# AzureLeon1/DiffSpectra

Hardware: AMD Instinct MI355X
Metric: molecules/sec, 1000-step QM9S all-spectra sampling (partial run) (higher is better)
Workload: dtype f32 (GEMMs as split-fp16 x3 MFMA with fp32 accumulate; fp32-level accuracy, parity gates unchanged)

## Files before the change

### __graft_entry__.py

```python
from __future__ import annotations

import os
import subprocess
import sys

ROOT = os.path.dirname(os.path.abspath(__file__))
if ROOT not in sys.path:
    sys.path.insert(0, ROOT)

CSRC = os.path.join(ROOT, "diffspectra_amd", "csrc")
HIP_SOURCES = [os.path.join(CSRC, n) for n in ("ds_forward.hip", "ds_gemm.hip", "ds_sampler.hip", "ds_spec.hip", "ds_aux.hip", "ds_match.hip", "ds_graph.hip", "ds_mces.hip", "ds_morgan.hip", "ds_subgeom.hip", "ds_mmd.hip", "ds_sets.hip", "ds_valence.hip", "ds_train.hip", "ds_train_gemm.hip", "ds_train_attn.hip", "ds_train_chain.hip")]
HIP_DEPS = [os.path.join(CSRC, "ds_device.h"), os.path.join(CSRC, "ds_host.h"), os.path.join(CSRC, "ds_train_common.h"), os.path.join(CSRC, "ds_svd3.h"), os.path.join(CSRC, "ds_records.h"), os.path.join(CSRC, "ds_bonds.h"),
            os.path.join(ROOT, "include", "diffspectra_hip.h"), os.path.join(ROOT, "include", "diffspectra_train.h"),
            os.path.join(ROOT, "include", "diffspectra_sets.h"), os.path.join(ROOT, "include", "diffspectra_valence.h")]
LIB = os.path.join(ROOT, "diffspectra_amd", "libdiffspectra_hip.so")
OBJ_DIR = os.path.join(ROOT, "build", "obj")
BASE_FLAGS = ["--offload-arch=gfx950", "-O3", "-std=c++17", "-fPIC", "-Wno-pass-failed", "-Wno-unused-value"]
OPT_FLAGS = ["-mllvm", "-amdgpu-mfma-vgpr-form=1"]
LIBRARY_STATE = "not built"


def _digest(paths):
    import hashlib
    h = hashlib.sha1()
    for p in paths:
        h.update(os.path.basename(p).encode() + b"\0")
        with open(p, "rb") as f:
            h.update(f.read())
    return h.hexdigest()


def _read(path):
    try:
        with open(path) as f:
            return f.read()
    except OSError:
        return None


def _stale(target, deps):
    return not os.path.exists(target) or any(not os.path.exists(d) for d in deps) or _read(target + ".src") != _digest(deps)


def _compile(hipcc, src, obj, flags):
    cmd = [hipcc, *flags, "-c", src, "-o", obj]
    print("[build]", " ".join(cmd), file=sys.stderr, flush=True)
    r = subprocess.run(cmd, cwd=ROOT, capture_output=True, text=True)
    if r.returncode != 0 and "Unknown command line argument" in r.stderr and any(f in flags for f in OPT_FLAGS):
        flags = [f for f in flags if f not in OPT_FLAGS]
        print("[build] this hipcc does not know -amdgpu-mfma-vgpr-form; retrying without it", file=sys.stderr, flush=True)
        return _compile(hipcc, src, obj, flags)
    if r.returncode != 0:
        sys.stderr.write(r.stderr)
        raise subprocess.CalledProcessError(r.returncode, cmd)
    with open(obj + ".flags", "w") as f:
        f.write(" ".join(flags))
    with open(obj + ".src", "w") as f:
        f.write(_digest([src] + HIP_DEPS))


def build(force: bool = False) -> None:
    from concurrent.futures import ThreadPoolExecutor
    hipcc = os.environ.get("HIPCC", "/opt/rocm/bin/hipcc")
    flags = BASE_FLAGS + OPT_FLAGS
    sources = [s for s in HIP_SOURCES if os.path.exists(s)]
    os.makedirs(OBJ_DIR, exist_ok=True)
    objs = [os.path.join(OBJ_DIR, os.path.basename(s)[:-4] + ".o") for s in sources]
# ... 63 lines not shown
```

### diffspectra_amd/abi.py

```python
from __future__ import annotations

import ctypes as C
import os
import re
import struct as _struct
from typing import Dict, List, NamedTuple, Tuple

_INCLUDE = os.path.join(os.path.dirname(os.path.dirname(os.path.abspath(__file__))), "include")

_FIELD_CODES = {"int64_t": "q", "int32_t": "i", "uint32_t": "I", "uint64_t": "Q", "float": "f"}
_CTYPES = {"P": C.c_void_p, "q": C.c_int64, "i": C.c_int32, "I": C.c_uint32, "Q": C.c_uint64, "f": C.c_float}
_ARG_CTYPES = {"*": C.c_void_p, "int": C.c_int, "int32_t": C.c_int32, "int64_t": C.c_int64, "uint32_t": C.c_uint32, "uint64_t": C.c_uint64,
               "float": C.c_float, "double": C.c_double}


class Prototype(NamedTuple):
    name: str
    ret: str
    params: List[Tuple[str, str]]

    @property
    def argtypes(self):
        return [_ARG_CTYPES[t] for _, t in self.params]

# ... 32 lines not shown
        self.prototypes = {name: Prototype(name, ret, self._params(name, params))
                           for ret, name, params in re.findall(r"^\s*(int|void)\s+(\w+)\s*\(([^()]*)\)\s*;", self.text, flags=re.M)}

    def _fields(self, body: str) -> List[Tuple[str, str]]:
        fields = []
        for decl in filter(None, (d.strip() for d in body.split(";"))):
            typ, rest = re.fullmatch(r"(?:const\s+)?(\w+)\s*(.*)", decl, flags=re.S).groups()
            for f_ in rest.split(","):
                name, length = re.fullmatch(r"([*\s]*\w+)\s*(?:\[\s*(\w+)\s*\])?", f_.strip()).groups()
                code = "P" if name.startswith("*") else _FIELD_CODES[typ]
                if length is not None:
                    code = f"{self.consts[length] if length in self.consts else int(length)}{code}"
                fields.append((name.lstrip("* "), code))
        return fields

    @staticmethod
    def _params(function: str, text: str) -> List[Tuple[str, str]]:
        params = []
        if text.strip() == "void":
            return params
        for decl in (d.strip() for d in text.split(",")):
            if "*" in decl:
                typ, m = "*", re.fullmatch(r"[\w\s*]*?(\w+)", decl)
            else:
                m = re.fullmatch(r"(?:const\s+)?(\w+)\s+(\w+)", decl)
                typ, m = (m.group(1), m) if m else (None, None)
            if m is None or typ not in _ARG_CTYPES:
                raise ValueError(f"{function}: parameter '{decl}' is neither a pointer nor one of the scalar types {sorted(_ARG_CTYPES)[1:]}")
            params.append((m.group(m.lastindex), typ))
        return params

    def exports(self, prefix: str) -> List[str]:
        return [name for name in self.prototypes if name.startswith(prefix)]

    def bind(self, lib: C.CDLL) -> None:
        for p in self.prototypes.values():
            fn = getattr(lib, p.name)
            fn.restype = None if p.ret == "void" else C.c_int
            fn.argtypes = p.argtypes

    def packer(self, name: str) -> _struct.Struct:
        return _struct.Struct("@" + "".join(code for _, code in self.structs[name]))

    def ctypes_struct(self, name: str):
        def ctype(code):
            return _CTYPES[code[-1]] * int(code[:-1]) if len(code) > 1 else _CTYPES[code]
        return type(name, (C.Structure,), {"_fields_": [(f_, ctype(code)) for f_, code in self.structs[name]]})


SAMPLING = Header("diffspectra_hip.h")
TRAINING = Header("diffspectra_train.h")
SETS = Header("diffspectra_sets.h")
VALENCE = Header("diffspectra_valence.h")
```

### diffspectra_amd/csrc/ds_forward.hip

```cpp
#include <hip/hip_runtime.h>
#include <math.h>
#include <stdint.h>
#include <stdlib.h>

#include <atomic>
#include <mutex>
#include <utility>
#include <vector>

#include "../../include/diffspectra_hip.h"
#include "ds_device.h"
#include "ds_host.h"

#define ADAC DS_ADA_COLS
constexpr int DS_NODE_PF = 8;
constexpr int DS_NODE_PF2 = 4;
constexpr int DS_QKV_PF = 4;
constexpr int DS_TWO_STREAM_MAX_PAIRS = 400000;

#ifdef DS_STAMPS
#define DS_STAMP_INIT()                                                                                 \
  unsigned long long _sa[16] = {0, 0, 0, 0, 0, 0, 0, 0, 0, 0, 0, 0, 0, 0, 0, 0};                        \
  unsigned long long _t0 = __builtin_amdgcn_s_memtime()
#define DS_STAMP(i)                                                                                     \
  do {                                                                                                  \
    const unsigned long long _t1 = __builtin_amdgcn_s_memtime();                                        \
    _sa[i] += _t1 - _t0;                                                                                \
    _t0 = _t1;                                                                                          \
  } while (0)
#define DS_STAMP_W(i)                                                                                   \
  do {                                                                                                  \
    asm volatile("s_waitcnt vmcnt(0) lgkmcnt(0)" ::: "memory");                                         \
    DS_STAMP(i);                                                                                        \
  } while (0)
#define DS_STAMP_FLUSH(t)                                                                               \
  do {                                                                                                  \
    if (threadIdx.x == (t))                                                                             \
      for (int _i = 0; _i < 16; ++_i)                                                                   \
        if (_sa[_i]) atomicAdd(reinterpret_cast<unsigned long long*>(c.ws.flags + 16) + _i, _sa[_i]);   \
  } while (0)
#else
#define DS_STAMP_INIT()
#define DS_STAMP(i)
#define DS_STAMP_W(i)
#define DS_STAMP_FLUSH(t)
#endif

namespace {

using dst::clear;
using dst::record;
using dst::wait;

struct Ctx {
  ds_layout L;
  ds_workspace ws;
  const float* wbase;
  const int64_t* woff;
  float edge_th, cutoff;
};

__device__ __forceinline__ const float* BW(const Ctx& c, int blk, int slot) {
  return c.wbase + c.woff[blk * DS_W_BLOCK_SLOTS + slot];
}
__device__ __forceinline__ const float* GW(const Ctx& c, int slot) {
  return c.wbase + c.woff[DS_NBLOCKS * DS_W_BLOCK_SLOTS + slot];
}

__device__ __forceinline__ float rbf_feature(float x, int k, const float* __restrict__ mean, const float* __restrict__ stdv,
                                             const float* __restrict__ astd) {
// ... 171 lines not shown
    const float* ade = c.ws.ada + blk * DS_ADA_BLOCK_STRIDE + DS_ADA_EDGE;
    const int lane = tid & 63, wv = tid >> 6;
#pragma unroll
    for (int j = 0; j < 4; ++j) {
      const float* am = ade + (size_t)rmol[16 * wv + 4 * j + (lane >> 4)] * ADAC;
      lsh[j] = reinterpret_cast<const float4*>(am)[lane & 15];
      lsc[j] = reinterpret_cast<const float4*>(am + 64)[lane & 15];
    }
  }
  {
    const int k = kf, rb = rbp;
    const float rsk = __builtin_amdgcn_rcpf(sk), rak = __builtin_amdgcn_rcpf(ak);
    const int Pp = c.L.Pp;
#pragma unroll
    for (int j = 0; j < 16; ++j) {
      const int row = rb + 4 * j, p = row0 + row;
      const float x = xs[row];
      const float z = (x - mk) * rsk;
      float v = k ? __expf(-0.5f * (z * z)) * rak : x;
      if (p >= Pp) { v = 0.0f; ev[j] = 0.0f; }
      split_store1(&Xh[row][0], 128, k, v);
      split_store1(&Xh[row][0], 128, 64 + k, ev[j]);
    }
  }
  {
    const int wv = tid >> 6, mt = wv >> 1, cc = wv & 1, lane = tid & 63;
    const WStreamH wse = wstream_h(BW(c, blk, DS_BW_EDGE_EMB_H), 64, 128, cc * 32);
    WRingH<8> ring;
    wring_h<8>(ring, wse, 0);
    const float bcol = BW(c, blk, DS_BW_EDGE_EMB_B)[cc * 32 + (lane & 31)];
    __syncthreads();
    f32x16 acc[1], lo[1];
#pragma unroll
    for (int i = 0; i < 16; ++i) acc[0][i] = bcol;
    acc_zero<1>(lo);
    wave_mma_h_deep<1, false, 8, 8>(&Xh[mt * 32][0], 128, wse, ring, 0, acc, lo);
    split_finish<1>(acc, lo);
#pragma unroll
    for (int i = 0; i < 16; ++i) Y[mt * 32 + acc_row(i, lane >> 5)][cc * 32 + (lane & 31)] = acc[0][i];
  }
  __syncthreads();
  {
    const int lane = tid & 63, wv = tid >> 6;
    _Float16* ye = reinterpret_cast<_Float16*>(c.ws.ye);
#pragma unroll
    for (int j = 0; j < 4; ++j) {
      const int row = 16 * wv + 4 * j + (lane >> 4);
      const float4 v = ln_mod_reg64(reinterpret_cast<const float4*>(&Y[row][0])[lane & 15], lsh[j], lsc[j]);
      if (row0 + row < c.L.Pp) split_store4(ye + (size_t)(row0 + row) * 128, 64, 4 * (lane & 15), v);
    }
  }
}

template <int NW>
__global__ __launch_bounds__(NW * 64) void k_node_qkv(Ctx c, int blk) {
  ds_fp16_saturate();
  constexpr int NT = NW * 64;
  constexpr int T = 64;
  constexpr int LDH = 2 * 256 + 8;
  __shared__ __attribute__((aligned(16))) _Float16 Xh[T][LDH];
  __shared__ int rmol[T];
  const int tid = threadIdx.x, row0 = blockIdx.x * T, col0 = blockIdx.y * 384;
  if (tid < T) rmol[tid] = (row0 + tid < c.L.Nn) ? c.L.node_mol[row0 + tid] : 0;
  __syncthreads();
  {
    const float* adn = c.ws.ada + blk * DS_ADA_BLOCK_STRIDE + DS_ADA_NODE;
    const int lane = tid & 63, wv = tid >> 6, g = lane >> 4, j = lane & 15;
    static_assert(NT == 256, "four waves x 16 rows");
#pragma unroll
    for (int half = 0; half < 2; ++half) {
      float4 v[2][4], sh[2][4], sc[2][4];
#pragma unroll
      for (int ps = 0; ps < 2; ++ps) {
        const int row = 16 * wv + 8 * half + 4 * ps + g;
        const float4* hp = reinterpret_cast<const float4*>(c.ws.h + (size_t)min(row0 + row, c.L.Nn - 1) * 256) + j;
        const float4* ap = reinterpret_cast<const float4*>(adn + (size_t)rmol[row] * ADAC) + j;
#pragma unroll
        for (int u = 0; u < 4; ++u) {
          v[ps][u] = hp[16 * u];
          sh[ps][u] = ap[16 * u];
          sc[ps][u] = ap[64 + 16 * u];
        }
      }
#pragma unroll
      for (int ps = 0; ps < 2; ++ps) {
        const int row = 16 * wv + 8 * half + 4 * ps + g;
        ln_mod_quad256(v[ps], sh[ps], sc[ps]);
#pragma unroll
        for (int u = 0; u < 4; ++u)
          split_store4(&Xh[row][0], 256, 64 * u + 4 * j, row0 + row < c.L.Nn ? v[ps][u] : make_float4(0, 0, 0, 0));
      }
    }
  }
  __syncthreads();
  const float* bias = BW(c, blk, DS_BW_QKV_B) + col0;
  float* qkv = c.ws.qkv + (size_t)row0 * 768 + col0;
  const int valid = c.L.Nn - row0, wave = tid >> 6;
  for (int ch = wave; ch < 12; ch += NW) {
    asm volatile("" ::: "memory");
    const float b = bias[ch * 32 + (tid & 31)];
    f32x16 acc[2], lo[2];
#pragma unroll
    for (int m = 0; m < 2; ++m)
#pragma unroll
      for (int i = 0; i < 16; ++i) acc[m][i] = b;
    acc_zero<2>(lo);
    wave_mma_h_ring<2, false, 16, DS_QKV_PF>(&Xh[0][0], 256, BW(c, blk, DS_BW_QKV_H), 768, 256, col0 + ch * 32, 0, acc, lo);
    split_finish<2>(acc, lo);
    acc_store<2, 768>(acc, qkv + ch * 32, valid, [](int, float v) { return v; });
  }
}

__global__ __launch_bounds__(1024) void k_attn_fused(Ctx c, int blk) {
  ds_fp16_saturate();
  DS_STAMP_INIT();
  constexpr int NT = 1024, QS = 512 + 32, LDT = 256 + 4, LDY = 2 * 64 + 8, CR = 32, MAXP = DS_MAX_ATOMS * (DS_MAX_ATOMS - 1) / 2;
  __shared__ __attribute__((aligned(16))) float QK[DS_MAX_ATOMS * QS];
  __shared__ __attribute__((aligned(16))) float Tt[2][CR][LDT];
  __shared__ __attribute__((aligned(16))) _Float16 Yc[2][CR][LDY];
  __shared__ __attribute__((aligned(16))) float AL[2][CR][32];
  __shared__ int PT[(MAXP + 15) & ~15];
  __shared__ int VT[32][32];
  static_assert(DS_MAX_ATOMS <= 32 && MAXP <= 511 - CR, "visit table packing");
  static_assert(DS_MAX_ATOMS * 128 <= 4 * NT && DS_MAX_ATOMS * 64 <= 2 * NT && MAXP <= NT, "single-pass staging");
  const int tid = threadIdx.x, wave = tid >> 6, lane = tid & 63, hh = lane >> 5;
  int n0, n, p0, P;
  if (c.L.mol_by_size) {
    const int4 r = reinterpret_cast<const int4*>(c.L.mol_by_size)[blockIdx.x];
    n0 = r.x; n = r.y; p0 = r.z; P = r.w;
  } else {
    const int m = blockIdx.x;
    n0 = c.L.node_off[m]; n = c.L.node_off[m + 1] - n0;
    p0 = c.L.pair_off[m]; P = c.L.pair_off[m + 1] - p0;
  }
  const WStreamH ws_e0 = wstream_h(BW(c, blk, DS_BW_E0_H), 256, 64, (wave & 7) * 32);
  const WStreamH ws_e1 = wstream_h(BW(c, blk, DS_BW_E1_H), 256, 64, (wave & 7) * 32);
  if (n <= 0) return;
  if (P <= 0) {
    for (int i = tid; i < 256; i += NT) c.ws.attn[(size_t)n0 * 256 + i] = 0.0f;
    return;
  }
  const int nch = (P + CR - 1) / CR;
  const bool producer = wave >= 8;
  const int ptid = tid & 511, prow = ptid >> 4, ppiece = ptid & 15;
  const u32x4* ye4 = reinterpret_cast<const u32x4*>(c.ws.ye) + (size_t)p0 * 16;
  auto row_pair = [&](int R) {
    const int d = R / n + 1, i = R - (d - 1) * n;
    int j = i + d;
    if (j >= n) j -= n;
    const int a = min(i, j), b = max(i, j);
    return a * (2 * n - a - 1) / 2 + (b - a - 1);
  };
  auto fetch_y = [&](int ck, bool class_order) {
    const int R = ck * CR + prow;
    const int Rc = min(R, P - 1);
    return ye4[(size_t)(class_order ? PT[Rc] : Rc) * 16 + ppiece];
  };
  auto commit_y = [&](int buf, const u32x4& v) { *reinterpret_cast<u32x4*>(&Yc[buf][prow][ppiece * 8]) = v; };
  h8 wf[2][4];
  auto load_weights = [&](const WStreamH& ws_) {
#pragma unroll
    for (int pl = 0; pl < 2; ++pl)
#pragma unroll
      for (int kb = 0; kb < 4; ++kb) wf[pl][kb] = wload_h(ws_, pl, kb);
// ... 425 lines not shown
      const int col = (wave + 4 * cc) * 32 + (tid & 31);
      const float gA = gAv[cc], gB = gBv[cc], bb = bbv[cc];
      const RowStore st = row_store<256>(c.ws.h + (size_t)row0 * 256 + (wave + 4 * cc) * 32);
#pragma unroll
      for (int i = 0; i < 16; ++i) {
        const int row = acc_row(i, hhl);
        float g = isB[i] ? gB : gA;
        if (!two) { const int m = rmol[row]; if (m != mA && m != mB) g = gsec[(size_t)m * ADAC + col]; }
        const float out = split_load1(&H2[row][0], 256, col) + g * (acc2[cc][0][i] + bb);
        split_store1(&H2[row][0], 256, col, out);
        if (row < rows_here) row_put(st, ((i & 3) + 8 * (i >> 2)) * 256 * 4, out);
      }
    }
  }
  __syncthreads();
  {
    const float* br = BW(c, blk, DS_BW_NODE_RO_B);
    auto ws_of = [&](int it) {
      return it < 2 ? wstream_h(BW(c, blk, DS_BW_NODE_RO_H), 64, 256, it * 32) : wstream_h(BW(c, blk, DS_BW_AC_H), 512, 256, (it - 2) * 32);
    };
    auto bias_of = [&](int it) { return it < 2 ? br[it * 32 + (tid & 31)] : 0.0f; };
    auto store_of = [&](int it, const f32x16 (&acc)[1]) {
      if (it < 2) acc_store<1, 768>(acc, c.ws.atom_hids + (size_t)row0 * 768 + 256 + 64 * blk + it * 32, Nn - row0, [](int, float v) { return v; });
      else acc_store<1, 512>(acc, c.ws.ac + (size_t)row0 * 512 + (it - 2) * 32, Nn - row0, [](int, float v) { return v; });
    };
#pragma unroll
    for (int pr = 0; pr < 2; ++pr) {
      asm volatile("" ::: "memory");
      const int itA = wave + 8 * pr, itB = itA + 4;
      f32x16 acc[2][1], lo[2][1];
      const float bA = bias_of(itA), bB = bias_of(itB);
#pragma unroll
      for (int i = 0; i < 16; ++i) { acc[0][0][i] = bA; acc[1][0][i] = bB; }
      acc_zero<1>(lo[0]); acc_zero<1>(lo[1]);
      wave_mma_h_ring_t2<1, false, 16, DS_NODE_PF2>(&H2[0][0], 256, ws_of(itA), ws_of(itB), 0, acc[0], lo[0], acc[1], lo[1]);
      split_finish<1>(acc[0], lo[0]);
      store_of(itA, acc[0]);
      split_finish<1>(acc[1], lo[1]);
      store_of(itB, acc[1]);
    }
    if (wave < 2) {
      asm volatile("" ::: "memory");
      const int it = 16 + wave;
      f32x16 acc[1], lo[1];
      acc_zero<1>(acc);
      acc_zero<1>(lo);
      wave_mma_h_ring<1, false, 16, DS_NODE_PF>(&H2[0][0], 256, BW(c, blk, DS_BW_AC_H), 512, 256, (it - 2) * 32, 0, acc, lo);
      split_finish<1>(acc, lo);
      store_of(it, acc);
    }
  }
}

__global__ __launch_bounds__(256, 2) void k_edge_update(Ctx c, int blk) {
  ds_fp16_saturate();
  DS_STAMP_INIT();
  constexpr int R = 32, LDW = 64 + DS_LDP;
  __shared__ __attribute__((aligned(16))) float E2s[4][R][LDW];
  __shared__ __attribute__((aligned(16))) float Ds[4][R][LDW];
  __shared__ int idx_s[4][3][R];
  const int tid = threadIdx.x, wave = tid >> 6, lane = tid & 63, hh = lane >> 5, r31 = lane & 31;
  constexpr int LDW2 = 2 * 64 + 8;
  float(*E2)[LDW] = E2s[wave];
  _Float16* E2h = reinterpret_cast<_Float16*>(&E2s[wave][0][0]);
  _Float16* Dh = reinterpret_cast<_Float16*>(&Ds[wave][0][0]);
  int* rmol = idx_s[wave][0];
  int* rpa = idx_s[wave][1];
  int* rpb = idx_s[wave][2];
  const int Pp = c.L.Pp;
  const int row0 = (blockIdx.x * 4 + wave) * R;
  if (row0 >= Pp) return;
  const int valid = min(R, Pp - row0);
  const float* ada = c.ws.ada + blk * DS_ADA_BLOCK_STRIDE + DS_ADA_EDGE;
  if (lane < R) {
    const int p = min(row0 + lane, Pp - 1);
    rmol[lane] = c.L.pair_mol[p]; rpa[lane] = c.L.pair_a[p]; rpb[lane] = c.L.pair_b[p];
  }
  DS_STAMP(0);
  {
    const float4* bn = reinterpret_cast<const float4*>(BW(c, blk, DS_BW_N2E_B));
    float rm[4], rs[4], ra[4];
#pragma unroll
    for (int t = 0; t < 4; ++t) {
      const int k = 4 * (lane & 15) + t;
      rm[t] = k ? BW(c, blk, DS_BW_RBF_MEAN)[k - 1] : 0.0f;
      rs[t] = __builtin_amdgcn_rcpf(k ? BW(c, blk, DS_BW_RBF_STD)[k - 1] : 1.0f);
      ra[t] = __builtin_amdgcn_rcpf(k ? BW(c, blk, DS_BW_RBF_ASTD)[k - 1] : 1.0f);
    }
#pragma unroll
    for (int it = 0; it < 2; ++it) {
      float4 ua[4], ub[4], ve[4], vd[4], vg[4], sh[4], sc[4];
      float xd[4];
#pragma unroll
      for (int u = 0; u < 4; ++u) {
        const int idx = lane + (it * 4 + u) * 64, row = idx >> 4, k4 = idx & 15;
        const size_t pc = (size_t)min(row0 + row, Pp - 1);
        const float* ad = ada + (size_t)rmol[row] * ADAC;
        ua[u] = reinterpret_cast<const float4*>(c.ws.u + (size_t)rpa[row] * 64)[k4];
        ub[u] = reinterpret_cast<const float4*>(c.ws.u + (size_t)rpb[row] * 64)[k4];
        ve[u] = reinterpret_cast<const float4*>(c.ws.e + pc * 64)[k4];
        xd[u] = c.ws.dist[pc];
        vg[u] = reinterpret_cast<const float4*>(ad + 128)[k4];
        sh[u] = reinterpret_cast<const float4*>(ad + 192)[k4];
        sc[u] = reinterpret_cast<const float4*>(ad + 256)[k4];
      }
#pragma unroll
// ... 655 lines not shown
  if (ctx) v += ctx[i];
  split_store1(reinterpret_cast<_Float16*>(c.ws.temb_silu) + b * 2048, 1024, (int)col, ds_silu(v));
}

bool make_ctx(Ctx& c, const ds_weights* w, const ds_layout* L, const ds_workspace* ws) {
  if (!w || !L || !ws || !w->base || !w->off_dev) return false;
  if (L->max_n > DS_MAX_ATOMS || L->B <= 0) return false;
  c.L = *L; c.ws = *ws; c.wbase = w->base; c.woff = w->off_dev;
  c.edge_th = w->edge_th; c.cutoff = w->spatial_cut_off;
  return true;
}

constexpr int MAX_DEVICES = 16;

inline int device_cus() {
  static std::atomic<int> cus[MAX_DEVICES];
  int dev = 0, n = 0;
  if (hipGetDevice(&dev) != hipSuccess || dev < 0 || dev >= MAX_DEVICES) return 256;
  if ((n = cus[dev].load(std::memory_order_relaxed)) > 0) return n;
  if (hipDeviceGetAttribute(&n, hipDeviceAttributeMultiprocessorCount, dev) != hipSuccess || n <= 0) n = 256;
  cus[dev].store(n, std::memory_order_relaxed);
  return n;
}

enum ProfSlot { PROF_EDGE_GEOM = 0, PROF_NODE_QKV = 1, PROF_ATTN = 2, PROF_NODE_UPDATE = 3, PROF_EDGE_UPDATE = 4, PROF_EQUI_PAIRS = 5 };
struct ProfState {
  int kernel = -1;
  int every = 1;
  long long seen = 0;
  std::vector<std::pair<hipEvent_t, hipEvent_t>> pool;
  size_t used = 0;
};
ProfState g_prof;

struct ProfScope {
  hipStream_t s;
  bool on = false;
  ProfScope(int kernel, hipStream_t st) : s(st) {
    if (g_prof.kernel != kernel) return;
    if ((g_prof.seen++ % g_prof.every) != 0 || g_prof.used >= g_prof.pool.size()) return;
    on = true;
    (void)hipEventRecord(g_prof.pool[g_prof.used].first, s);
  }
  ~ProfScope() {
    if (on) (void)hipEventRecord(g_prof.pool[g_prof.used++].second, s);
  }
};

void launch_edge_geom(const Ctx& c, int blk, hipStream_t s) {
  if (c.L.Pp <= 0) return;
  ProfScope ps(PROF_EDGE_GEOM, s);
  hipLaunchKernelGGL(k_edge_geom, dim3((c.L.Pp + 63) / 64), dim3(256), 0, s, c, blk);
}
void launch_node_qkv(const Ctx& c, int blk, hipStream_t s) {
  ProfScope ps(PROF_NODE_QKV, s);
  hipLaunchKernelGGL(k_node_qkv<4>, dim3((c.L.Nn + 63) / 64, 2), dim3(256), 0, s, c, blk);
}
void launch_attn(const Ctx& c, int blk, hipStream_t s) {
  ProfScope ps(PROF_ATTN, s);
  hipLaunchKernelGGL(k_attn_fused, dim3(c.L.B), dim3(1024), 0, s, c, blk);
}
void launch_node_n2e(const Ctx& c, int blk, hipStream_t s) { hipLaunchKernelGGL(k_node_n2e, dim3((c.L.Nn + 63) / 64), dim3(256), 0, s, c, blk); }
template <bool N2E>
void launch_node_update(const Ctx& c, int blk, hipStream_t s) {
  ProfScope ps(PROF_NODE_UPDATE, s);
  hipLaunchKernelGGL(k_node_update<N2E>, dim3((c.L.Nn + 31) / 32), dim3(256), 0, s, c, blk);
}
void launch_edge_update(const Ctx& c, int blk, hipStream_t s) {
  if (c.L.Pp <= 0) return;
  ProfScope ps(PROF_EDGE_UPDATE, s);
  hipLaunchKernelGGL(k_edge_update, dim3((c.L.Pp + 127) / 128), dim3(256), 0, s, c, blk);
}
void launch_equi_pairs(const Ctx& c, int blk, hipStream_t s) {
  if (c.L.Pp <= 0) return;
  ProfScope ps(PROF_EQUI_PAIRS, s);
  hipLaunchKernelGGL(k_equi_pairs, dim3(min((c.L.Pp + 31) / 32, device_cus())), dim3((EQUI_NCW + EQUI_NLW) * 64), 0, s, c, blk);
}
void launch_pos_update(const Ctx& c, int last, hipStream_t s) { hipLaunchKernelGGL(k_pos_update, dim3(c.L.B), dim3(64), 0, s, c, last); }

}

extern "C" {

void ds_struct_sizes(int64_t* out) {
  out[0] = sizeof(ds_weights);
  out[1] = sizeof(ds_layout);
  out[2] = sizeof(ds_workspace);
  out[3] = sizeof(ds_gemm_args);
}

int ds_stage_time(const ds_weights* w, const ds_layout* L, ds_workspace* ws, const float* noise_level, const float* ctx_emb,
                  void* stream) {
  hipStream_t s = (hipStream_t)stream;
  Ctx c;
  if (!make_ctx(c, w, L, ws) || !noise_level) return DS_ERR_ARG;
  const int B = L->B;
  const int64_t* off = w->off + DS_NBLOCKS * DS_W_BLOCK_SLOTS;
  hipLaunchKernelGGL(k_time_feat, dim3((B + 63) / 64), dim3(64), 0, s, c, noise_level);
  ds_gemm_args g{};
  g.A = ws->tfeat; g.lda = 24; g.Wp = w->base + off[DS_GW_TM1_W]; g.bias = w->base + off[DS_GW_TM1_B];
  g.C = ws->tmid; g.ldc = 1024; g.M = B; g.K = 24; g.N = 1024; g.act = 2;
  int st = ds_gemm(&g, stream);
  if (st) return st;
  float* tm3 = ws->ada;
  g.A = ws->tmid; g.lda = 1024; g.Wp = w->base + off[DS_GW_TM3_W]; g.bias = w->base + off[DS_GW_TM3_B];
  g.C = tm3; g.K = 1024; g.act = 0;
  st = ds_gemm(&g, stream);
  if (st) return st;
  const size_t tot = (size_t)B * 1024;
  hipLaunchKernelGGL(k_temb_finish, dim3((unsigned)((tot + 255) / 256)), dim3(256), 0, s, c, (const float*)tm3, B, ctx_emb);
  static_assert(ADAC % 32 == 0, "adaLN table width");
  return ds_gemm_split(ws->temb_silu, w->base + off[DS_GW_ADA_W], w->base + off[DS_GW_ADA_B], ws->ada, ADAC, B, 1024, ADAC, stream);
}

int ds_stage_init(const ds_weights* w, const ds_layout* L, ds_workspace* ws, const float* xh, const float* edge_x,
                  const float* cond_x, const float* cond_edge_x, void* stream) {
  hipStream_t s = (hipStream_t)stream;
  Ctx c;
  if (!make_ctx(c, w, L, ws) || !xh || !edge_x || ((cond_x == nullptr) != (cond_edge_x == nullptr))) return DS_ERR_ARG;
// ... 34 lines not shown
  hipStream_t s = nullptr;
  hipEvent_t fork[DS_NBLOCKS + 1] = {}, join[DS_NBLOCKS + 1] = {};
  std::once_flag once;
  bool ok = false;
};
static SideStream g_side[MAX_DEVICES];
static int g_two_stream = -1;

static SideStream* side_stream() {
  int dev = 0;
  if (hipGetDevice(&dev) != hipSuccess || dev < 0 || dev >= MAX_DEVICES) return nullptr;
  SideStream& ss = g_side[dev];
  std::call_once(ss.once, [&ss] {
    bool ok = hipStreamCreateWithFlags(&ss.s, hipStreamNonBlocking) == hipSuccess;
    for (int i = 0; ok && i <= DS_NBLOCKS; ++i)
      ok = hipEventCreateWithFlags(&ss.fork[i], hipEventDisableTiming) == hipSuccess &&
           hipEventCreateWithFlags(&ss.join[i], hipEventDisableTiming) == hipSuccess;
    ss.ok = ok;
  });
  return ss.ok ? &ss : nullptr;
}

static int forward_blocks_two_streams(const ds_weights* w, const ds_layout* L, ds_workspace* ws, hipStream_t s, SideStream* ss) {
  Ctx c;
  if (!make_ctx(c, w, L, ws)) return DS_ERR_ARG;
  hipStream_t s2 = ss->s;
  const hipEvent_t fork0 = ss->fork[DS_NBLOCKS], join0 = ss->join[DS_NBLOCKS];
  if (!record(fork0, s) || !wait(s2, fork0)) return DS_ERR_LAUNCH;
  launch_node_qkv(c, 0, s2);
  if (!record(join0, s2)) return DS_ERR_LAUNCH;
  for (int blk = 0; blk < DS_NBLOCKS; ++blk) {
    launch_edge_geom(c, blk, s);
    if (!wait(s, blk == 0 ? join0 : ss->join[blk - 1])) return DS_ERR_LAUNCH;
    launch_attn(c, blk, s);
    launch_node_n2e(c, blk, s);
    if (!record(ss->fork[blk], s) || !wait(s2, ss->fork[blk])) return DS_ERR_LAUNCH;
    launch_node_update<false>(c, blk, s2);
    if (blk + 1 < DS_NBLOCKS) launch_node_qkv(c, blk + 1, s2);
    if (!record(ss->join[blk], s2)) return DS_ERR_LAUNCH;
    launch_edge_update(c, blk, s);
    if (!wait(s, ss->join[blk])) return DS_ERR_LAUNCH;
    launch_equi_pairs(c, blk, s);
    launch_pos_update(c, blk == DS_NBLOCKS - 1 ? 1 : 0, s);
  }
  return DST_CHECK_LAUNCH();
}

int ds_set_two_stream(int on) {
  const int prev = g_two_stream;
  g_two_stream = on;
  return prev;
}

int ds_forward(const ds_weights* w, const ds_layout* L, ds_workspace* ws, const float* xh, const float* edge_x,
               const float* cond_x, const float* cond_edge_x, const float* noise_level, const float* ctx_emb, float* out_xh,
               float* out_edge, void* stream) {
  int st = ds_stage_time(w, L, ws, noise_level, ctx_emb, stream);
  if (st) return st;
  st = ds_stage_init(w, L, ws, xh, edge_x, cond_x, cond_edge_x, stream);
  if (st) return st;
  static const int env_two = [] { const char* e = getenv("DIFFSPECTRA_TWO_STREAM"); return e ? atoi(e) : -1; }();
  const int pick = g_two_stream >= 0 ? g_two_stream : env_two;
  const int two = pick >= 0 ? pick : (L->Pp < DS_TWO_STREAM_MAX_PAIRS ? 1 : 0);
  SideStream* ss = two ? side_stream() : nullptr;
  if (ss) {
    st = forward_blocks_two_streams(w, L, ws, (hipStream_t)stream, ss);
    if (st) return st;
  } else {
    for (int b = 0; b < DS_NBLOCKS; ++b) {
      st = ds_stage_block(w, L, ws, b, b == DS_NBLOCKS - 1, stream);
      if (st) return st;
    }
  }
  return ds_stage_readout(w, L, ws, out_xh, out_edge, stream);
}

int ds_profile_config(int kernel, int every, int max_samples) {
  for (auto& e : g_prof.pool) { (void)hipEventDestroy(e.first); (void)hipEventDestroy(e.second); }
  g_prof.pool.clear();
  g_prof.used = 0; g_prof.seen = 0;
  g_prof.kernel = kernel; g_prof.every = every > 0 ? every : 1;
  if (kernel < 0) return DS_OK;
  if (kernel > 6 || max_samples <= 0) return DS_ERR_ARG;
  g_prof.pool.resize((size_t)max_samples);
  for (auto& e : g_prof.pool)
    if (hipEventCreate(&e.first) != hipSuccess || hipEventCreate(&e.second) != hipSuccess) return DS_ERR_LAUNCH;
  return DS_OK;
}

int ds_profile_read(double* total_ms, int64_t* samples) {
  if (!total_ms || !samples) return DS_ERR_ARG;
  double tot = 0.0;
  for (size_t i = 0; i < g_prof.used; ++i) {
    float ms = 0.0f;
    if (hipEventSynchronize(g_prof.pool[i].second) != hipSuccess) return DS_ERR_LAUNCH;
    if (hipEventElapsedTime(&ms, g_prof.pool[i].first, g_prof.pool[i].second) != hipSuccess) return DS_ERR_LAUNCH;
    tot += ms;
  }
  *total_ms = tot; *samples = (int64_t)g_prof.used;
  g_prof.used = 0; g_prof.seen = 0;
  return DS_OK;
}

}
```

### diffspectra_amd/engine.py

```python
from __future__ import annotations

import ctypes as C
import os
from typing import Dict, List, Optional

import numpy as np
import torch

from . import abi
from .abi import ptr

_ptr = ptr

LIB_PATH = os.environ.get("DIFFSPECTRA_HIP_LIB", os.path.join(os.path.dirname(os.path.abspath(__file__)), "libdiffspectra_hip.so"))

_HDR = abi.SAMPLING
HEADER_PATH = _HDR.path
CONSTS = _HDR.consts
BLOCK_SLOTS, GLOBAL_SLOTS = _HDR.enums["ds_block_slot"], _HDR.enums["ds_global_slot"]
EXPORTS = _HDR.exports("ds_")
NB = CONSTS["DS_NBLOCKS"]
W_BLOCK_SLOTS, W_GLOBAL_SLOTS, W_NUM_SLOTS = CONSTS["DS_W_BLOCK_SLOTS"], CONSTS["DS_W_GLOBAL_SLOTS"], CONSTS["DS_W_NUM_SLOTS"]
ADA_COLS = CONSTS["DS_ADA_COLS"]
ADA_STRIDE = CONSTS["DS_ADA_BLOCK_STRIDE"]
MAX_ATOMS = CONSTS["DS_MAX_ATOMS"]

DsWeights = _HDR.ctypes_struct("ds_weights")
DsLayout = _HDR.ctypes_struct("ds_layout")
DsWorkspace = _HDR.ctypes_struct("ds_workspace")
DsGemmArgs = _HDR.ctypes_struct("ds_gemm_args")
_WS_FIELDS = [f for f, _ in _HDR.structs["ds_workspace"]]

_lib = None


def load_library() -> C.CDLL:
    global _lib
    if _lib is not None:
        return _lib
    if not os.path.exists(LIB_PATH):
        raise RuntimeError(f"{LIB_PATH} is missing: build it with `python -c 'import __graft_entry__ as g; g.build()'`. "
                           "diffspectra_amd has no CPU/PyTorch fallback.")
    lib = C.CDLL(LIB_PATH)
    abi.SAMPLING.bind(lib)
    abi.TRAINING.bind(lib)
    abi.SETS.bind(lib)
    abi.VALENCE.bind(lib)
    sizes = (C.c_int64 * 4)()
    lib.ds_struct_sizes(sizes)
    mine = [C.sizeof(t) for t in (DsWeights, DsLayout, DsWorkspace, DsGemmArgs)]
    if list(sizes) != mine:
        raise RuntimeError(f"C-ABI struct layout mismatch: library {list(sizes)} vs binding {mine}")
    _lib = lib
    return lib


def _check(status: int, what: str):
    if status != 0:
        raise RuntimeError(f"{what} failed with status {status} "
                           f"({ {-1: 'bad argument', -2: 'HIP launch error'}.get(status, 'unknown')})")


def _stream():
    return torch.cuda.current_stream().cuda_stream


def _f32c(t: torch.Tensor, device) -> torch.Tensor:
    return t.detach().to(device=device, dtype=torch.float32).contiguous()



def pack_linear(weight: torch.Tensor, n_pad_to: int = 32) -> torch.Tensor:
    w = weight.detach().to(torch.float32).cpu()
    N, K = w.shape
    Kp, Np = (K + 7) // 8 * 8, (N + n_pad_to - 1) // n_pad_to * n_pad_to
    b = torch.zeros(Kp, Np)
    b[:K, :N] = w.t()
    return b.view(Kp // 8, 2, 4, Np).permute(0, 1, 3, 2).contiguous().reshape(-1)


SPLIT_SCALE = 2048.0
TANH_PRESCALE = 2.8853900817779268
F16_MAX = 65504.0


def _check_split_range(w: torch.Tensor, what: str) -> None:
    m = float(w.abs().max()) if w.numel() else 0.0
    if not (m < F16_MAX):
        raise ValueError(f"{what}: max |w| = {m:.4g} is outside the split-fp16 range (|w| < {F16_MAX:g}); "
                         "this weight cannot run on the f16 matrix pipe")



def pack_linear_f16_split(weight: torch.Tensor) -> torch.Tensor:
    w = weight.detach().to(torch.float32).cpu()
    _check_split_range(w, "pack_linear_f16_split")
    if w.shape[0] % 32:
        w = torch.cat([w, torch.zeros(32 - w.shape[0] % 32, w.shape[1])], 0)
    N, K = w.shape
    assert K % 16 == 0
# ... 739 lines not shown
```

Before: 233.1.

## Add 64-row, 512-thread node QKV and node-update kernels for large batches

Measured after the change: 235.8 (median of 6 runs). +1.1%, better.

```diff
diff --git a/__graft_entry__.py b/__graft_entry__.py
--- a/__graft_entry__.py
+++ b/__graft_entry__.py
@@ -12,7 +12,7 @@
 HIP_SOURCES = [os.path.join(CSRC, n) for n in ("ds_forward.hip", "ds_gemm.hip", "ds_sampler.hip", "ds_spec.hip", "ds_aux.hip", "ds_match.hip", "ds_graph.hip", "ds_mces.hip", "ds_morgan.hip", "ds_subgeom.hip", "ds_mmd.hip", "ds_sets.hip", "ds_valence.hip", "ds_train.hip", "ds_train_gemm.hip", "ds_train_attn.hip", "ds_train_chain.hip")]
 HIP_DEPS = [os.path.join(CSRC, "ds_device.h"), os.path.join(CSRC, "ds_host.h"), os.path.join(CSRC, "ds_train_common.h"), os.path.join(CSRC, "ds_svd3.h"), os.path.join(CSRC, "ds_records.h"), os.path.join(CSRC, "ds_bonds.h"),
             os.path.join(ROOT, "include", "diffspectra_hip.h"), os.path.join(ROOT, "include", "diffspectra_train.h"),
-            os.path.join(ROOT, "include", "diffspectra_sets.h"), os.path.join(ROOT, "include", "diffspectra_valence.h")]
+            os.path.join(ROOT, "include", "diffspectra_sets.h"), os.path.join(ROOT, "include", "diffspectra_valence.h"), os.path.join(ROOT, "include", "diffspectra_tiles.h")]
 LIB = os.path.join(ROOT, "diffspectra_amd", "libdiffspectra_hip.so")
 OBJ_DIR = os.path.join(ROOT, "build", "obj")
 BASE_FLAGS = ["--offload-arch=gfx950", "-O3", "-std=c++17", "-fPIC", "-Wno-pass-failed", "-Wno-unused-value"]
diff --git a/diffspectra_amd/abi.py b/diffspectra_amd/abi.py
--- a/diffspectra_amd/abi.py
+++ b/diffspectra_amd/abi.py
@@ -108,3 +108,4 @@
 TRAINING = Header("diffspectra_train.h")
 SETS = Header("diffspectra_sets.h")
 VALENCE = Header("diffspectra_valence.h")
+TILES = Header("diffspectra_tiles.h")
diff --git a/diffspectra_amd/csrc/ds_forward.hip b/diffspectra_amd/csrc/ds_forward.hip
--- a/diffspectra_amd/csrc/ds_forward.hip
+++ b/diffspectra_amd/csrc/ds_forward.hip
@@ -9,6 +9,7 @@
 #include <vector>
 
 #include "../../include/diffspectra_hip.h"
+#include "../../include/diffspectra_tiles.h"
 #include "ds_device.h"
 #include "ds_host.h"
 
@@ -16,6 +17,8 @@
 constexpr int DS_NODE_PF = 8;
 constexpr int DS_NODE_PF2 = 4;
 constexpr int DS_QKV_PF = 4;
+constexpr int DS_QKV_PF_WIDE = 4;
+constexpr int DS_NODE_TILE64_MIN_PER_CU = 4;
 constexpr int DS_TWO_STREAM_MAX_PAIRS = 400000;
 
 #ifdef DS_STAMPS
@@ -293,11 +296,12 @@
   }
 }
 
-template <int NW>
-__global__ __launch_bounds__(NW * 64) void k_node_qkv(Ctx c, int blk) {
+template <int NW, int PF>
+__device__ __forceinline__ void node_qkv_tile(const Ctx& c, int blk) {
   ds_fp16_saturate();
-  constexpr int NT = NW * 64;
   constexpr int T = 64;
+  constexpr int RW = T / NW;
+  constexpr int NCH = 3 * NW;
   constexpr int LDH = 2 * 256 + 8;
   __shared__ __attribute__((aligned(16))) _Float16 Xh[T][LDH];
   __shared__ int rmol[T];
@@ -307,13 +311,13 @@
   {
     const float* adn = c.ws.ada + blk * DS_ADA_BLOCK_STRIDE + DS_ADA_NODE;
     const int lane = tid & 63, wv = tid >> 6, g = lane >> 4, j = lane & 15;
-    static_assert(NT == 256, "four waves x 16 rows");
-#pragma unroll
-    for (int half = 0; half < 2; ++half) {
+    static_assert(NW == 4 || NW == 8, "four waves x 16 rows or eight waves x 8 rows");
+#pragma unroll
+    for (int half = 0; half < RW / 8; ++half) {
       float4 v[2][4], sh[2][4], sc[2][4];
 #pragma unroll
       for (int ps = 0; ps < 2; ++ps) {
-        const int row = 16 * wv + 8 * half + 4 * ps + g;
+        const int row = RW * wv + 8 * half + 4 * ps + g;
         const float4* hp = reinterpret_cast<const float4*>(c.ws.h + (size_t)min(row0 + row, c.L.Nn - 1) * 256) + j;
         const float4* ap = reinterpret_cast<const float4*>(adn + (size_t)rmol[row] * ADAC) + j;
 #pragma unroll
@@ -325,7 +329,7 @@
       }
 #pragma unroll
       for (int ps = 0; ps < 2; ++ps) {
-        const int row = 16 * wv + 8 * half + 4 * ps + g;
+        const int row = RW * wv + 8 * half + 4 * ps + g;
         ln_mod_quad256(v[ps], sh[ps], sc[ps]);
 #pragma unroll
         for (int u = 0; u < 4; ++u)
@@ -337,7 +341,7 @@
   const float* bias = BW(c, blk, DS_BW_QKV_B) + col0;
   float* qkv = c.ws.qkv + (size_t)row0 * 768 + col0;
   const int valid = c.L.Nn - row0, wave = tid >> 6;
-  for (int ch = wave; ch < 12; ch += NW) {
+  for (int ch = wave; ch < NCH; ch += NW) {
     asm volatile("" ::: "memory");
     const float b = bias[ch * 32 + (tid & 31)];
     f32x16 acc[2], lo[2];
@@ -346,11 +350,13 @@
 #pragma unroll
       for (int i = 0; i < 16; ++i) acc[m][i] = b;
     acc_zero<2>(lo);
-    wave_mma_h_ring<2, false, 16, DS_QKV_PF>(&Xh[0][0], 256, BW(c, blk, DS_BW_QKV_H), 768, 256, col0 + ch * 32, 0, acc, lo);
+    wave_mma_h_ring<2, false, 16, PF>(&Xh[0][0], 256, BW(c, blk, DS_BW_QKV_H), 768, 256, col0 + ch * 32, 0, acc, lo);
     split_finish<2>(acc, lo);
     acc_store<2, 768>(acc, qkv + ch * 32, valid, [](int, float v) { return v; });
   }
 }
+__global__ __launch_bounds__(256) void k_node_qkv(Ctx c, int blk) { node_qkv_tile<4, DS_QKV_PF>(c, blk); }
+__global__ __launch_bounds__(512, 2) void k_node_qkv_wide(Ctx c, int blk) { node_qkv_tile<8, DS_QKV_PF_WIDE>(c, blk); }
 
 __global__ __launch_bounds__(1024) void k_attn_fused(Ctx c, int blk) {
   ds_fp16_saturate();
@@ -882,6 +888,200 @@
   }
 }
 
+constexpr int DS_GATE_SLOTS = 16;
+template <bool N2E>
+__global__ __launch_bounds__(512) void k_node_update64(Ctx c, int blk) {
+  ds_fp16_saturate();
+  constexpr int T = 64, LDH = 2 * 256 + 8, GS = DS_GATE_SLOTS;
+  __shared__ __attribute__((aligned(16))) _Float16 B1[T][LDH];
+  __shared__ __attribute__((aligned(16))) _Float16 H2[T][LDH];
+  __shared__ __attribute__((aligned(16))) float G[GS][256];
+  __shared__ int rmol[T], rslot[T], smol[T], nslot;
+  const int tid = threadIdx.x, wave = tid >> 6, row0 = blockIdx.x * T;
+  const int Nn = c.L.Nn;
+  const float* ada = c.ws.ada;
+  const float* gsec = ada + blk * DS_ADA_BLOCK_STRIDE + DS_ADA_NODE + 1280;
+  float4 va[2][4], vh[2][4];
+#pragma unroll
+  for (int ps = 0; ps < 2; ++ps) {
+    const size_t gr = (size_t)min(row0 + 8 * wave + 4 * ps + ((tid & 63) >> 4), Nn - 1);
+    const float4* ap = reinterpret_cast<const float4*>(c.ws.attn + gr * 256) + (tid & 15);
+    const float4* hp = reinterpret_cast<const float4*>(c.ws.h + gr * 256) + (tid & 15);
+#pragma unroll
+    for (int u = 0; u < 4; ++u) {
+      va[ps][u] = ap[16 * u];
+      vh[ps][u] = hp[16 * u];
+    }
+  }
+  if (tid < T) {
+    const bool in = row0 + tid < Nn;
+    const int m = in ? c.L.node_mol[row0 + tid] : 0;
+    const bool first = in && (tid == 0 || c.L.node_mol[row0 + tid - 1] != m);
+    const unsigned long long starts = __ballot(first);
+    const int slot = __popcll(starts & ((2ull << tid) - 1ull)) - 1;
+    rmol[tid] = m;
+    rslot[tid] = slot;
+    if (first) smol[slot] = m;
+    if (tid == 0) nslot = __popcll(starts);
+  }
+  __syncthreads();
+  const int ns = nslot;
+  {
+    const int lane = tid & 63, g = lane >> 4, j = lane & 15;
+    float4 vg[2][4], sh[2][4], sc[2][4], gv[2];
+#pragma unroll
+    for (int ps = 0; ps < 2; ++ps) {
+      const int row = 8 * wave + 4 * ps + g;
+      const float4* ad = reinterpret_cast<const float4*>(ada + (size_t)rmol[row] * ADAC + blk * DS_ADA_BLOCK_STRIDE + DS_ADA_NODE) + j;
+#pragma unroll
+      for (int u = 0; u < 4; ++u) {
+        vg[ps][u] = ad[128 + 16 * u];
+        sh[ps][u] = ad[192 + 16 * u];
+        sc[ps][u] = ad[256 + 16 * u];
+      }
+    }
+#pragma unroll
+    for (int u = 0; u < 2; ++u)
+      gv[u] = reinterpret_cast<const float4*>(gsec + (size_t)smol[min(wave + 8 * u, ns - 1)] * ADAC)[lane];
+#pragma unroll
+    for (int ps = 0; ps < 2; ++ps) {
+      const int row = 8 * wave + 4 * ps + g;
+      float4 r[4];
+#pragma unroll
+      for (int u = 0; u < 4; ++u) {
+        if (row0 + row >= Nn) va[ps][u] = vh[ps][u] = make_float4(0, 0, 0, 0);
+        if (N2E) split_store4(&B1[row][0], 256, 64 * u + 4 * j, va[ps][u]);
+        r[u].x = vh[ps][u].x + vg[ps][u].x * va[ps][u].x; r[u].y = vh[ps][u].y + vg[ps][u].y * va[ps][u].y;
+        r[u].z = vh[ps][u].z + vg[ps][u].z * va[ps][u].z; r[u].w = vh[ps][u].w + vg[ps][u].w * va[ps][u].w;
+      }
+      ln_mod_quad256(r, sh[ps], sc[ps]);
+#pragma unroll
+      for (int u = 0; u < 4; ++u) split_store4(&H2[row][0], 256, 64 * u + 4 * j, r[u]);
+    }
+#pragma unroll
+    for (int u = 0; u < 2; ++u) reinterpret_cast<float4*>(&G[wave + 8 * u][0])[lane] = gv[u];
+  }
+  const float* W1 = BW(c, blk, DS_BW_FF1_H);
+  const float* W2 = BW(c, blk, DS_BW_FF2_H);
+  auto tail_ws = [&](int it) {
+    return it < 2 ? wstream_h(BW(c, blk, DS_BW_NODE_RO_H), 64, 256, it * 32) : wstream_h(BW(c, blk, DS_BW_AC_H), 512, 256, (it - 2) * 32);
+  };
+  WRingH<DS_NODE_PF> ring, ring_n2e;
+  const bool n2e = N2E && wave < 4 && row0 + (wave >> 1) * 32 < Nn;
+  const WStreamH wsn = wstream_h(BW(c, blk, DS_BW_N2E_H), 64, 256, (wave & 1) * 32);
+  if (n2e) wring_h<DS_NODE_PF>(ring_n2e, wsn, 0);
+  wring_h<DS_NODE_PF>(ring, wstream_h(W1, 512, 256, wave * 32), 0);
+  __syncthreads();
+  if (N2E) {
+    {
+      const int mt = wave >> 1, cc = wave & 1;
+      if (n2e) {
+        f32x16 acc[1], lo[1];
+        acc_zero<1>(acc);
+        acc_zero<1>(lo);
+        wave_mma_h_deep<1, false, 16, DS_NODE_PF>(&B1[mt * 32][0], 256, wsn, ring_n2e, 0, acc, lo);
+        split_finish<1>(acc, lo);
+        acc_store<1, 64>(acc, c.ws.u + (size_t)(row0 + mt * 32) * 64 + cc * 32, Nn - row0 - mt * 32, [](int, float v) { return v; });
+      }
+    }
+    __syncthreads();
+  }
+  {
+    const float* b1 = BW(c, blk, DS_BW_FF1_B);
+    const WStreamH ws2 = wstream_h(W2, 256, 512, wave * 32);
+    f32x16 acc2[2], lo2[2];
+    acc_zero<2>(acc2);
+    acc_zero<2>(lo2);
+    const int col = wave * 32 + (tid & 31);
+    const float bb = BW(c, blk, DS_BW_FF2_B)[col];
+    for (int half = 0; half < 2; ++half) {
+      {
+        asm volatile("" ::: "memory");
+        const int hhf = (tid & 63) >> 5;
+        f32x16 acc[2], lo[2];
+        const float bf = b1[half * 256 + col];
+#pragma unroll
+        for (int m = 0; m < 2; ++m)
+#pragma unroll
+          for (int i = 0; i < 16; ++i) acc[m][i] = bf;
+        acc_zero<2>(lo);
+        wave_mma_h_deep<2, false, 16, DS_NODE_PF>(&H2[0][0], 256, wstream_h(W1, 512, 256, (half * 8 + wave) * 32), ring, 0, acc, lo);
+        wring_h<DS_NODE_PF>(ring, ws2, half * 16);
+        split_finish<2>(acc, lo);
+#pragma unroll
+        for (int m = 0; m < 2; ++m)
+#pragma unroll
+          for (int i = 0; i < 16; i += 2) {
+            f32x2 v;
+            v.x = acc[m][i]; v.y = acc[m][i + 1];
+            v = ds_silu2(v);
+            const int r0 = m * 32 + acc_row(i, hhf);
+            split_store1(&B1[r0][0], 256, col, v.x);
+            split_store1(&B1[r0 + 1][0], 256, col, v.y);
+          }
+      }
+      __syncthreads();
+      asm volatile("" ::: "memory");
+      wave_mma_h_deep<2, false, 16, DS_NODE_PF>(&B1[0][0], 256, ws2, ring, half * 16, acc2, lo2, half * 16);
+      wring_h<DS_NODE_PF>(ring, half == 0 ? wstream_h(W1, 512, 256, (8 + wave) * 32) : tail_ws(wave), 0);
+      __syncthreads();
+    }
+    split_finish<2>(acc2, lo2);
+    float* Gx = reinterpret_cast<float*>(&B1[0][0]);
+    if (ns > GS) {
+      for (int idx = tid; idx < (ns - GS) * 64; idx += 512)
+        reinterpret_cast<float4*>(Gx)[idx] = reinterpret_cast<const float4*>(gsec + (size_t)smol[GS + (idx >> 6)] * ADAC)[idx & 63];
+      __syncthreads();
+    }
+    const int hhl = (tid & 63) >> 5;
+    const int rows_here = Nn - row0;
+    const RowStore st = row_store<256>(c.ws.h + (size_t)row0 * 256 + wave * 32);
+#pragma unroll
+    for (int m = 0; m < 2; ++m)
+#pragma unroll
+      for (int i = 0; i < 16; ++i) {
+        const int row = m * 32 + acc_row(i, hhl), s = rslot[row];
+        const float g = s < GS ? G[s][col] : Gx[(s - GS) * 256 + col];
+        const float out = split_load1(&H2[row][0], 256, col) + g * (acc2[m][i] + bb);
+        split_store1(&H2[row][0], 256, col, out);
+        if (row < rows_here) row_put(st, (m * 32 + (i & 3) + 8 * (i >> 2)) * 256 * 4, out);
+      }
+  }
+  __syncthreads();
+  {
+    const float* br = BW(c, blk, DS_BW_NODE_RO_B);
+    const int mt = (wave >> 1) & 1, itl = 16 + (wave & 1);
+    const bool last = wave >= 4 && row0 + mt * 32 < Nn;
+#pragma unroll
+    for (int pr = 0; pr < 2; ++pr) {
+      asm volatile("" ::: "memory");
+      const int it = wave + 8 * pr;
+      const float bi = it < 2 ? br[it * 32 + (tid & 31)] : 0.0f;
+      f32x16 acc[2], lo[2];
+#pragma unroll
+      for (int m = 0; m < 2; ++m)
+#pragma unroll
+        for (int i = 0; i < 16; ++i) acc[m][i] = bi;
+      acc_zero<2>(lo);
+      wave_mma_h_deep<2, false, 16, DS_NODE_PF>(&H2[0][0], 256, tail_ws(it), ring, 0, acc, lo);
+      if (pr == 0) wring_h<DS_NODE_PF>(ring, tail_ws(wave + 8), 0);
+      else if (last) wring_h<DS_NODE_PF>(ring, tail_ws(itl), 0);
+      split_finish<2>(acc, lo);
+      if (it < 2) acc_store<2, 768>(acc, c.ws.atom_hids + (size_t)row0 * 768 + 256 + 64 * blk + it * 32, Nn - row0, [](int, float v) { return v; });
+      else acc_store<2, 512>(acc, c.ws.ac + (size_t)row0 * 512 + (it - 2) * 32, Nn - row0, [](int, float v) { return v; });
+    }
+    if (last) {
+      asm volatile("" ::: "memory");
+      f32x16 acc[1], lo[1];
+      acc_zero<1>(acc);
+      acc_zero<1>(lo);
+      wave_mma_h_deep<1, false, 16, DS_NODE_PF>(&H2[mt * 32][0], 256, tail_ws(itl), ring, 0, acc, lo);
+      split_finish<1>(acc, lo);
+      acc_store<1, 512>(acc, c.ws.ac + (size_t)(row0 + mt * 32) * 512 + (itl - 2) * 32, Nn - row0 - mt * 32, [](int, float v) { return v; });
+    }
+  }
+}
+
 __global__ __launch_bounds__(256, 2) void k_edge_update(Ctx c, int blk) {
   ds_fp16_saturate();
   DS_STAMP_INIT();
@@ -1643,9 +1843,17 @@
   ProfScope ps(PROF_EDGE_GEOM, s);
   hipLaunchKernelGGL(k_edge_geom, dim3((c.L.Pp + 63) / 64), dim3(256), 0, s, c, blk);
 }
+int g_node_tile = -1;
+bool node_tile64(const Ctx& c) {
+  static const int env_tile = [] { const char* e = getenv("DIFFSPECTRA_NODE_TILE"); return e ? atoi(e) : -1; }();
+  const int pick = g_node_tile > 0 ? g_node_tile : env_tile;
+  if (pick == 32 || pick == 64) return pick == 64;
+  return (c.L.Nn + 63) / 64 >= DS_NODE_TILE64_MIN_PER_CU * device_cus();
+}
 void launch_node_qkv(const Ctx& c, int blk, hipStream_t s) {
   ProfScope ps(PROF_NODE_QKV, s);
-  hipLaunchKernelGGL(k_node_qkv<4>, dim3((c.L.Nn + 63) / 64, 2), dim3(256), 0, s, c, blk);
+  if (node_tile64(c)) hipLaunchKernelGGL(k_node_qkv_wide, dim3((c.L.Nn + 63) / 64), dim3(512), 0, s, c, blk);
+  else hipLaunchKernelGGL(k_node_qkv, dim3((c.L.Nn + 63) / 64, 2), dim3(256), 0, s, c, blk);
 }
 void launch_attn(const Ctx& c, int blk, hipStream_t s) {
   ProfScope ps(PROF_ATTN, s);
@@ -1655,7 +1863,8 @@
 template <bool N2E>
 void launch_node_update(const Ctx& c, int blk, hipStream_t s) {
   ProfScope ps(PROF_NODE_UPDATE, s);
-  hipLaunchKernelGGL(k_node_update<N2E>, dim3((c.L.Nn + 31) / 32), dim3(256), 0, s, c, blk);
+  if (node_tile64(c)) hipLaunchKernelGGL(k_node_update64<N2E>, dim3((c.L.Nn + 63) / 64), dim3(512), 0, s, c, blk);
+  else hipLaunchKernelGGL(k_node_update<N2E>, dim3((c.L.Nn + 31) / 32), dim3(256), 0, s, c, blk);
 }
 void launch_edge_update(const Ctx& c, int blk, hipStream_t s) {
   if (c.L.Pp <= 0) return;
@@ -1796,6 +2005,12 @@
   return prev;
 }
 
+int ds_set_node_tile(int rows) {
+  const int prev = g_node_tile;
+  g_node_tile = (rows == 32 || rows == 64) ? rows : -1;
+  return prev;
+}
+
 int ds_forward(const ds_weights* w, const ds_layout* L, ds_workspace* ws, const float* xh, const float* edge_x,
                const float* cond_x, const float* cond_edge_x, const float* noise_level, const float* ctx_emb, float* out_xh,
                float* out_edge, void* stream) {
diff --git a/diffspectra_amd/engine.py b/diffspectra_amd/engine.py
--- a/diffspectra_amd/engine.py
+++ b/diffspectra_amd/engine.py
@@ -46,6 +46,7 @@
     abi.TRAINING.bind(lib)
     abi.SETS.bind(lib)
     abi.VALENCE.bind(lib)
+    abi.TILES.bind(lib)
     sizes = (C.c_int64 * 4)()
     lib.ds_struct_sizes(sizes)
     mine = [C.sizeof(t) for t in (DsWeights, DsLayout, DsWorkspace, DsGemmArgs)]
diff --git a/include/diffspectra_tiles.h b/include/diffspectra_tiles.h
--- /dev/null
+++ b/include/diffspectra_tiles.h
@@ -0,0 +1,13 @@
+#ifndef DIFFSPECTRA_TILES_H
+#define DIFFSPECTRA_TILES_H
+
+#ifdef __cplusplus
+extern "C" {
+#endif
+
+int ds_set_node_tile(int rows);
+
+#ifdef __cplusplus
+}
+#endif
+#endif
```
